# NVlabs/STEP

Hardware: AMD Instinct MI355X
Metric: clips_per_sec_T32_224 (higher is better)
Workload: dtype bf16; 1 GPU; C2: I3D backbone (BaseNet conv3d_1a..mixed_4f) forward, 8 x [3,32,224,224] clips per GPU, inputs resident in HBM, random-init weights; clips_per_gpu=8, T=32, HW=224, parallelism=clip-sharded replicas x1 (no data-path collective), batches_in_flight=2

## Files before the change

include/step_amd.h:

```cpp
#ifndef STEP_AMD_H
#define STEP_AMD_H

#include <stddef.h>
#include <stdint.h>

#ifdef __cplusplus
extern "C" {
#endif

#define STEP_API __attribute__((visibility("default")))

typedef void* step_stream_t;

enum { STEP_F32 = 0, STEP_BF16 = 1, STEP_F16 = 2 };
enum { STEP_NCHW = 0, STEP_NHWC = 1 };

enum {
    STEP_OK = 0,
    STEP_E_DTYPE = -1,
    STEP_E_SHAPE = -2,
    STEP_E_NULL = -3,
    STEP_E_UNSUPPORTED = -4,
    STEP_E_ALIGN = -5
};
// ... 8 lines not shown
STEP_API int step_hbm_stream_probe(const void* src, void* dst, size_t bytes, int workgroups, step_stream_t stream);

enum {
    STEP_OPT_CONV_IMPL = 0,
    STEP_OPT_CONV_NB,
    STEP_OPT_CONV_WAVES,
    STEP_OPT_CONV_PHASED,
    STEP_OPT_CONV_GEN,
    STEP_OPT_CONV_GMODE,
    STEP_OPT_CONV_PWS,
    STEP_OPT_CONV_SPLITK,
    STEP_OPT_CONV_TAIL,
    STEP_OPT_CONV_SLOTS,
    STEP_OPT_POOL_DIRECT,
    STEP_OPT_WGRAD_MINPIX,
    STEP_OPT_WGRAD16_LDS,
    STEP_OPT_CONV_GROUP_PW,
    STEP_OPT_CLIP_VEC,
    STEP_OPT_CONV_NB_RULE,
    STEP_OPT_THROUGHPUT,
    STEP_OPT_CONV_PERSIST,
    STEP_OPT_CONV_PWS_WAVES,
    STEP_OPT_CONV_GROUP_NARROW,
    STEP_OPT_COUNT_
};
STEP_API int step_set_option(int option, int value);
STEP_API int step_get_option(int option, int* value);
STEP_API void step_reset_options(void);
STEP_API const char* step_option_name(int option);

STEP_API int step_roi_align_forward(const void* feat, int dtype, int layout, const float* rois, int K, int B,
                                    int C, int H, int W, int pooled_h, int pooled_w, float spatial_scale,
                                    int sampling_ratio, void* out, step_stream_t stream);

STEP_API int step_roi_align_tubes_forward(const void* feat, int dtype, const float* rois, int K, int B, int T_all, int T, int C,
                                          int H, int W, int pooled_h, int pooled_w, float spatial_scale, int sampling_ratio,
                                          void* out, step_stream_t stream);

#define STEP_ROI_BWD_GATHER 0
#define STEP_ROI_BWD_ATOMIC 1
STEP_API int step_roi_align_backward(const float* grad, int layout, const float* rois, int K, int B, int C, int H,
                                     int W, int pooled_h, int pooled_w, float spatial_scale, int sampling_ratio,
                                     int mode, float* grad_feat, step_stream_t stream);

STEP_API int step_roi_pool_forward(const void* feat, int dtype, int layout, const float* rois, int K, int B, int C,
                                   int H, int W, int pooled_h, int pooled_w, float spatial_scale, void* out,
// ... 48 lines not shown
STEP_API size_t step_conv_packed_elems(int Cout, int Cin, int kd, int kh, int kw);
STEP_API int step_conv_pack_weight(const float* w, int Cout, int Cin, int kd, int kh, int kw, int dtype,
                                   const int32_t* perm_c, void* packed, step_stream_t stream);
STEP_API int step_conv_pack_weight_dgrad(const float* w, int Cout, int Cin, int kd, int kh, int kw, int dtype, int cin_pad,
                                         void* packed, step_stream_t stream);
typedef struct step_pack_item {
    const float* w;
    const int32_t* perm_c;
    void* packed;
    int Cout, Cin, w_cin, cin_lo;
    int kd, kh, kw;
    int dgrad, cin_pad;
    int reserved;
} step_pack_item;
STEP_API int step_conv_pack_weights(const step_pack_item* items, int n, int dtype, step_stream_t stream);
STEP_API int step_conv_forward(const step_conv_desc* d, const void* x, const void* w_packed, const float* scale,
                               const float* shift, const void* res, void* y, void* y2, step_stream_t stream);

STEP_API int step_pool_conv_forward(int dtype, const void* x, int N, int D, int H, int W, int C, int x_cstride, int x_coff, void* pool_y,
                                    int py_cstride, int py_coff, const step_conv_desc* d, const void* cx, const void* w_packed,
                                    const float* scale, const float* shift, void* y, void* y2, step_stream_t stream);

STEP_API int step_pool_conv_plan_nb(const step_conv_desc* d);

STEP_API int step_conv_forward_cat(const step_conv_desc* d, const void* x, int cin_a, const void* xb, int xb_cstride, int xb_coff,
                                   const void* w_packed, const float* scale, const float* shift, const void* res, void* y, void* y2,
                                   step_stream_t stream);

STEP_API int step_conv_forward_pre(const step_conv_desc* d, const void* x, const void* w_packed, const float* scale, const float* shift,
                                   const void* pre_w_packed, const float* pre_scale, const float* pre_shift, int pre_cin, void* y,
                                   step_stream_t stream);

STEP_API size_t step_conv_pre_pool_workspace_bytes(const step_conv_desc* d);
STEP_API int step_conv_forward_pre_pool(const step_conv_desc* d, const void* x, const void* w_packed, const float* scale, const float* shift,
                                        const void* pre_w_packed, const float* pre_scale, const float* pre_shift, int pre_cin, void* y_pooled,
                                        void* ws, size_t ws_bytes, step_stream_t stream);
STEP_API int step_conv_forward_pre_pool_tiles(const step_conv_desc* d, const void* x, const void* w_packed, const float* scale, const float* shift,
                                              const void* pre_w_packed, const float* pre_scale, const float* pre_shift, int pre_cin, void* y_pooled,
                                              void* ws, size_t ws_bytes, step_stream_t stream);
STEP_API int step_conv_pre_pool_finish(const step_conv_desc* d, void* y_pooled, void* ws, size_t ws_bytes, step_stream_t stream);

typedef struct step_conv_item {
    const step_conv_desc* desc;
    const void* x; const void* w_packed; const float* scale; const float* shift; const void* res; void* y;
} step_conv_item;
STEP_API int step_conv_forward_group(const step_conv_item* items, int n, step_stream_t stream);
// ... 227 lines not shown
```

step_amd/_capi.py:

```python
import ctypes as C

F32, BF16, F16 = 0, 1, 2
NCHW, NHWC = 0, 1
ROI_BWD_GATHER, ROI_BWD_ATOMIC = 0, 1
ABI_VERSION = 48

vp, fp, ip, u8p = C.c_void_p, C.c_void_p, C.c_void_p, C.c_void_p
i, f, ll, sz = C.c_int, C.c_float, C.c_longlong, C.c_size_t


class ConvDesc(C.Structure):
    _fields_ = [(n, C.c_int) for n in (
        "dtype", "N", "D", "H", "W", "Cin", "Cout", "kd", "kh", "kw", "x_cstride", "x_coff", "y_cstride", "y_coff",
        "res_cstride", "res_coff", "relu", "split", "y2_cstride", "y2_coff")]


class PackItem(C.Structure):
    _fields_ = [("w", C.c_void_p), ("perm_c", C.c_void_p), ("packed", C.c_void_p)] + [(n, C.c_int) for n in (
        "Cout", "Cin", "w_cin", "cin_lo", "kd", "kh", "kw", "dgrad", "cin_pad", "reserved")]


class ConvItem(C.Structure):
    _fields_ = [("desc", C.POINTER(ConvDesc)), ("x", C.c_void_p), ("w_packed", C.c_void_p), ("scale", C.c_void_p), ("shift", C.c_void_p),
                ("res", C.c_void_p), ("y", C.c_void_p)]


class WgradReduceItem(C.Structure):
    _fields_ = [("ws", C.c_void_p), ("dw", C.c_void_p), ("jobs", C.c_longlong)] + [(n, C.c_int) for n in (
# ... 16 lines not shown
    "step_roi_pool_backward": (i, [fp, ip, i, fp, i, i, i, i, i, i, i, fp, vp]),
    "step_mfma_clock_probe": (i, [vp, i, i, vp]),
    "step_hbm_stream_probe": (i, [vp, vp, sz, i, vp]),
    "step_clock_sample": (i, [vp, i, i, vp]),
    "step_nms_scratch_bytes": (sz, [i, i]),
    "step_nms_batched": (i, [fp, fp, ip, i, i, f, u8p, vp, vp]),
    "step_nms_batched_f64": (i, [fp, fp, ip, i, i, f, u8p, vp, vp]),
    "step_detect_compact": (i, [u8p, vp, vp, vp, ip, i, i, i, i, f, f, fp, fp, vp, vp, ip, vp]),
    "step_detect_merge": (i, [fp, ip, ip, ip, i, i, f, ip, ip, fp, ip, vp]),
    "step_round_sig4": (i, [fp, ll, fp, ip, vp]),
    "step_eval_match": (i, [fp, ip, vp, fp, ip, vp, i, ll, ll, i, C.c_double, u8p, ip, vp]),
    "step_eval_ap": (i, [vp, u8p, vp, i, ll, fp, fp, fp, vp]),
    "step_detect_nms": (i, [fp, ll, i, fp, ll, ip, ip, i, i, f, f, f, f, u8p, fp, vp]),
    "step_conv_packed_elems": (sz, [i, i, i, i, i]),
    "step_conv_pack_weight": (i, [fp, i, i, i, i, i, i, ip, vp, vp]),
    "step_conv_pack_weight_dgrad": (i, [fp, i, i, i, i, i, i, i, vp, vp]),
    "step_conv_pack_weights": (i, [vp, i, i, vp]),
    "step_conv_forward": (i, [C.POINTER(ConvDesc), vp, vp, fp, fp, vp, vp, vp, vp]),
    "step_conv_forward_group": (i, [C.POINTER(ConvItem), i, vp]),
    "step_conv_group_kernel_name": (i, [C.POINTER(ConvItem), i, C.c_char_p, i]),
    "step_conv_workspace_bytes": (sz, [C.POINTER(ConvDesc)]),
    "step_pool_conv_forward": (i, [i, vp, i, i, i, i, i, i, i, vp, i, i, C.POINTER(ConvDesc), vp, vp, fp, fp, vp, vp, vp]),
    "step_pool_conv_plan_nb": (i, [C.POINTER(ConvDesc)]),
    "step_conv_forward_cat": (i, [C.POINTER(ConvDesc), vp, i, vp, i, i, vp, fp, fp, vp, vp, vp, vp]),
    "step_conv_forward_pre": (i, [C.POINTER(ConvDesc), vp, vp, fp, fp, vp, fp, fp, i, vp, vp]),
    "step_conv_pre_pool_workspace_bytes": (sz, [C.POINTER(ConvDesc)]),
    "step_conv_forward_pre_pool": (i, [C.POINTER(ConvDesc), vp, vp, fp, fp, vp, fp, fp, i, vp, vp, sz, vp]),
    "step_conv_forward_pre_pool_tiles": (i, [C.POINTER(ConvDesc), vp, vp, fp, fp, vp, fp, fp, i, vp, vp, sz, vp]),
    "step_conv_pre_pool_finish": (i, [C.POINTER(ConvDesc), vp, vp, sz, vp]),
    "step_conv_wgrad": (i, [C.POINTER(ConvDesc), vp, fp, fp, i, vp]),
    "step_conv_wgrad_workspace_bytes": (sz, [C.POINTER(ConvDesc)]),
    "step_conv_wgrad_ws": (i, [C.POINTER(ConvDesc), vp, fp, fp, i, vp, sz, vp]),
    "step_conv_wgrad16": (i, [C.POINTER(ConvDesc), vp, vp, fp, i, vp]),
    "step_conv_wgrad16_workspace_bytes": (sz, [C.POINTER(ConvDesc)]),
    "step_conv_wgrad16_ws": (i, [C.POINTER(ConvDesc), vp, vp, fp, i, vp, sz, vp]),
    "step_conv_wgrad_kernel_name": (i, [C.POINTER(ConvDesc), i, C.c_char_p, i]),
    "step_conv_wgrad_partial": (i, [C.POINTER(ConvDesc), vp, vp, i, fp, i, vp, sz, C.POINTER(WgradReduceItem), vp]),
    "step_wgrad_reduce_group": (i, [C.POINTER(WgradReduceItem), i, vp]),
    "step_conv_forward_ws": (i, [C.POINTER(ConvDesc), vp, vp, fp, fp, vp, vp, vp, vp, sz, vp]),
    "step_conv_kernel_name": (i, [C.POINTER(ConvDesc), C.c_char_p, i]),
    "step_conv_plan_info": (i, [C.POINTER(ConvDesc), C.POINTER(C.c_int), i]),
    "step_conv_pre_pool_plan_info": (i, [C.POINTER(ConvDesc), C.POINTER(C.c_int), i]),
    "step_stem_packed_elems": (sz, [i]),
    "step_stem_pack_weight": (i, [fp, i, i, vp, vp]),
    "step_stem_forward": (i, [i, vp, i, i, i, i, vp, fp, fp, i, i, vp, i, i, vp]),
    "step_stem_pool_workspace_bytes": (sz, [i, i, i, i, i, i]),
# ... 50 lines not shown

def declare(lib, strict=True):
    for name, (res, args) in SIGNATURES.items():
        if not strict and not hasattr(lib, name):
            continue
        fn = getattr(lib, name)
        fn.restype = res
        fn.argtypes = args
    return lib


_ERR = {-1: "unsupported dtype", -2: "bad shape", -3: "null pointer", -4: "unsupported configuration",
        -5: "misaligned pointer or channel count"}


def check(status, what):
    if status != 0:
        msg = _ERR.get(status, "hipError_t %d" % status) if status < 0 else "hipError_t %d" % status
        raise RuntimeError("%s failed: %s" % (what, msg))


OPTION_IDS = {name: k for k, name in enumerate((
    "conv_impl", "conv_nb", "conv_waves", "conv_phased", "conv_gen", "conv_gmode", "conv_pws", "conv_splitk", "conv_tail",
    "conv_slots", "pool_direct", "wgrad_minpix", "wgrad16_lds", "conv_group_pw", "clip_vec", "conv_nb_rule", "throughput", "conv_persist", "conv_pws_waves", "conv_group_narrow"))}


def set_option(lib, name, value):
    check(lib.step_set_option(OPTION_IDS[name], int(value)), "step_set_option(%s, %r)" % (name, value))


def get_option(lib, name):
    v = C.c_int()
    check(lib.step_get_option(OPTION_IDS[name], C.byref(v)), "step_get_option(%s)" % name)
    return v.value


class options:

    def __init__(self, lib, **kw):
        self.lib, self.kw = lib, kw

    def __enter__(self):
        self.prev = {k: get_option(self.lib, k) for k in self.kw}
        for k, v in self.kw.items():
            set_option(self.lib, k, v)
        return self

# ... 5 lines not shown
```

step_amd/backbone.py:

```python
import os
import weakref

import torch
import torch.nn as nn

from . import ops, wgrad
from .wgrad import STATE as WGRAD, wgrad_into_grad, wgrad_sync

BN_EPS = 1e-5

MIXED_CFG = {
    "3b": (192, (64, 96, 128, 16, 32, 32)), "3c": (256, (128, 128, 192, 32, 96, 64)),
    "4b": (480, (192, 96, 208, 16, 48, 64)), "4c": (512, (160, 112, 224, 24, 64, 64)),
    "4d": (512, (128, 128, 256, 24, 64, 64)), "4e": (512, (112, 144, 288, 32, 64, 64)),
    "4f": (528, (256, 160, 320, 32, 128, 128)), "5b": (832, (256, 160, 320, 32, 128, 128)),
    "5c": (832, (384, 192, 384, 48, 128, 128)),
}


def _ver(*tensors):
    return tuple((t.data_ptr(), t._version, t.device) for t in tensors if t is not None)


class _ConvUnitFn(torch.autograd.Function):
# ... 650 lines not shown
        grad = torch.is_grad_enabled() and (x.requires_grad or any(p.requires_grad for p in self.parameters()))
        bn_train = any(u._unit.bn_training for u in (self.branch_0, self.branch_1[0], self.branch_1[1], self.branch_2[0], self.branch_2[1], self.branch_3[1]))
        if grad and not bn_train and self._train_fn_ok(x):
            u0, u1a, u1b, u2a, u2b, u3 = self._train_units()
            y = _MixedTrainFn.apply(x, u0.weight_fn(), u1a.weight_fn(), u1b.weight_fn(), u2a.weight_fn(), u2b.weight_fn(), u3.weight_fn(), self)
            if out is not None:
                out.copy_(y)
                return out
            return y
        if grad or bn_train:
            y = torch.cat([self.branch_0(x), self.branch_1[1](self.branch_1[0](x)), self.branch_2[1](self.branch_2[0](x)),
                           self.branch_3[1](self.branch_3[0](x))], dim=-1)
            if out is not None:
                out.copy_(y)
                return out
            return y
        if out is None:
            out = torch.empty((N, D, H, W, self.out_channels), dtype=x.dtype, device=x.device)
        c0, c1, c2 = oc[0], oc[0] + oc[2], oc[0] + oc[2] + oc[4]
        t = torch.empty((N, D, H, W, oc[1] + oc[3]), dtype=x.dtype, device=x.device)
        if BRANCH_STREAMS == 0 or not x.is_cuda:
            pool = self.branch_3[0]
            p = self._fused(x, out[..., :c0], t, pool=POOL_WITH_POINTWISE and pool.kernel_size == (3, 3, 3) and pool.stride == (1, 1, 1))
            if p is None:
                p = pool(x)
            u1, u2, u3 = self.branch_1[1]._unit, self.branch_2[1]._unit, self.branch_3[1]._unit
            m = []
            for u, xin, o in ((u1, t[..., :oc[1]], out[..., c0:c1]), (u2, t[..., oc[1]:], out[..., c1:c2]), (u3, p, out[..., c2:])):
                scale, shift = u.affine()
                m.append((xin, u.packed(x.dtype), u.cout, u.k, scale, None if shift is None else shift.detach().contiguous(), True, o))
            ops.conv_forward_group(m)
            return out
        main = torch.cuda.current_stream(x.device)
        s1, s2 = WGRAD.side_streams(x.device)
        if BRANCH_STREAMS == 1:
            s1 = s2
        s2.wait_stream(main)
        with torch.cuda.stream(s2):
            p = self._branch_3(x, out[..., c2:])
        self._fused(x, out[..., :c0], t)
        s1.wait_stream(main)
        with torch.cuda.stream(s1):
            self.branch_2[1](t[..., oc[1]:], out=out[..., c1:c2])
        self.branch_1[1](t[..., :oc[1]], out=out[..., c0:c1])
        main.wait_stream(s1)
        if s2 is not s1:
            main.wait_stream(s2)
        if p is not None:
            p.record_stream(main)
        return out

    def _branch_3(self, x, out):
        pool, unit = self.branch_3[0], self.branch_3[1]
        p = pool(x)
        unit(p, out=out)
        return p


POOL_WITH_POINTWISE = True
FUSE_STEM_POOL = True
FUSE_STEM_U8 = False
FUSE_CONV_POOL = True
FUSE_POINTWISE_INPUT = True


def _stem_then_pool(a, b, x, u8=None):
    if not (isinstance(a, Unit3D) and a.is_stem and isinstance(b, MaxPoolTF)) or not x.is_cuda or x.dtype == torch.float32:
        return None
    if b.kernel_size != (1, 3, 3) or b.stride != (1, 2, 2) or not a.relu or a._unit.bn_training or a._unit.bn is None:
        return None
    w = a.conv3d.weight
    bn = a.batch3d
    if torch.is_grad_enabled() and (w.requires_grad or bn.weight.requires_grad or bn.bias.requires_grad or x.requires_grad):
        return None
    scale, shift = a._unit.affine()
    if u8 is not None:
        dtype, mode, mean, std = u8
        return ops.stem_pool_forward_u8(x, dtype, a.stem_packed(dtype), w.shape[0], scale, shift, mode, mean, std)
    return ops.stem_pool_forward(x, a.stem_packed(x.dtype), w.shape[0], scale, shift)


def _pointwise_then_3x3x3(a, b, x, pool=None):
# ... 223 lines not shown
```

step_amd/csrc/conv_common.h:

```cpp
#pragma once
#include "options.h"
#include "common.h"
#include <stdio.h>
#include <stdlib.h>
#include <type_traits>
#include <utility>

namespace step {


constexpr int CK = 32;

__host__ __device__ constexpr int taps_padded(int ntaps) { return (ntaps > 1 && (ntaps & 1)) ? ntaps + 1 : ntaps; }

struct ConvParams {
    const void* x; const void* w; const float* scale; const float* shift; const void* res; void* y; void* y2;
    int split, y2_cstride, y2_coff;
    int N, D, H, W, Cin, Cout;
    int x_cstride, x_coff, y_cstride, y_coff, r_cstride, r_coff;
    int relu;
    int tiles_h, tiles_w, tiles_d;
    int gtd, gth, gtw;
    int gmode;
    int gx, gy;
    int gbase, gcount;
    int tile0;
    const void* x2; int x2_cstride, x2_coff, s_split;
    int gpersist;
    int narrow;
    int nchunks;
    int nchunks32;
    int vec_epi;
    int nblk32;
    long long Mtot;
    unsigned mag_hhw, mag_hw;
    const void* pre_w; const float* pre_scale; const float* pre_shift;
    void* pool_row; void* pool_col; int Hp, Wp;
    int pool_p2;
#ifdef STEP_PROBE
    unsigned long long* probe;
#endif
};

int pool333_pw_launch(int dtype, const void* x, int N, int D, int H, int W, int C, int x_cstride, int x_coff, void* y, int y_cstride, int y_coff,
                      ConvParams cp, long long conv_blocks, int nbc, step_stream_t stream);

constexpr int CONV_GROUP_MAX = 2;
struct ConvGroupParams { ConvParams p[CONV_GROUP_MAX]; int n; ConvParams pw; };

#ifdef STEP_PROBE
extern unsigned long long* g_probe_buf;
__device__ __forceinline__ void probe_mark(unsigned long long* probe, int slot) {
    if (probe && threadIdx.x == 0) probe[(size_t)blockIdx.x * 16 + slot] = __builtin_amdgcn_s_memrealtime();
}
__device__ __forceinline__ void probe_clock_begin(unsigned long long* probe) {
    if (probe && threadIdx.x == 0) probe[(size_t)blockIdx.x * 16 + 14] = __builtin_amdgcn_s_memtime();
}
__device__ __forceinline__ void probe_clock_end(unsigned long long* probe) {
    if (probe && threadIdx.x == 0) probe[(size_t)blockIdx.x * 16 + 14] = __builtin_amdgcn_s_memtime() - probe[(size_t)blockIdx.x * 16 + 14];
}
__device__ __forceinline__ void probe_ids(unsigned long long* probe) {
    probe_clock_begin(probe);
    if (probe && threadIdx.x == 0) {
        const unsigned hw = __builtin_amdgcn_s_getreg((31 << 11) | 4);
        const unsigned xcc = __builtin_amdgcn_s_getreg((31 << 11) | 20);
        probe[(size_t)blockIdx.x * 16 + 15] = ((unsigned long long)xcc << 32) | hw;
    }
}
#define STEP_PROBE_MARK(p, slot) probe_mark((p).probe, slot)
// ... 135 lines not shown
```

step_amd/csrc/conv_igemm.hip:

```cpp
#include "conv_common.h"

namespace step {

template <typename T, int TWL, int NB, int KD, int KH, int KW, bool FLAT, int CKT>
__global__ __launch_bounds__(256) void conv_igemm_kernel(ConvParams p) {
    constexpr int TW = 1 << TWL, TH = 128 >> TWL;
    constexpr int HH_ = TH + KH - 1, HW_ = TW + KW - 1;
    constexpr int NPIX = FLAT ? 128 : KD * HH_ * HW_;
    constexpr int ES = (int)sizeof(T);
    constexpr int VEC = 16 / ES;
    constexpr int PITCH = CKT * ES;
    constexpr int KSTEPS = CKT / 16;
    constexpr int SLOTS = PITCH / 16;
    constexpr int PPR = (16 / SLOTS) > 0 ? (16 / SLOTS) : 1;
    constexpr int NTAPS = KD * KH * KW;
    constexpr int NVEC = NPIX * SLOTS;
    constexpr int ITER = (NVEC + 255) / 256;
    typedef typename Ld16<T>::type vec16;
    typedef typename frag<T>::type frag_t;

    constexpr int LDSB = (NPIX * PITCH > 16384) ? NPIX * PITCH : 16384;
    __shared__ __attribute__((aligned(16))) unsigned char lds[LDSB];

    const int tid = threadIdx.x;
// ... 764 lines not shown
    step_conv_desc canon;
    ConvParams p;
    const int rc = conv_fill_params(d, cx, w_packed, scale, shift, nullptr, y, y2, canon, p);
    if (rc != STEP_OK) return rc;
    if (N == 0 && p.N == 0) return STEP_OK;
    if (!x || !pool_y) return STEP_E_NULL;
    if (N == 0 || p.N == 0 || canon.dtype != dtype || dtype == STEP_F32 || !(canon.kd == 1 && canon.kh == 1 && canon.kw == 1)) return STEP_E_UNSUPPORTED;
    constexpr int VEC = 8;
    if (canon.Cin % VEC || canon.x_cstride % VEC || canon.x_coff % VEC || ((uintptr_t)p.x % 16) || ((uintptr_t)p.w % 16) || ((uintptr_t)x % 16) ||
        ((uintptr_t)pool_y % 16))
        return STEP_E_UNSUPPORTED;
    const ConvPlan pl = conv_plan(&canon, false);
    if (!pl.ok || pl.impl != 2 || pl.NB > 2) return STEP_E_UNSUPPORTED;
    p.tiles_h = pl.tiles_h; p.tiles_w = pl.tiles_w; p.tiles_d = pl.tiles_d;
    p.gtd = pl.gtd; p.gth = pl.gth; p.gtw = pl.gtw; p.gmode = pl.gmode;
    const long long mtiles = ceil_div64(p.Mtot, 128);
    const int nbc = pool_conv_nbc(pl, p.Mtot, p.nblk32);
    const int groups = ceil_div(p.nblk32, 2 * nbc);
    p.gx = (int)mtiles; p.gy = groups;
    const long long tot = (mtiles * groups + 7) / 8 * 8;
    return pool333_pw_launch(dtype, x, N, D, H, W, C, x_cstride, x_coff, pool_y, py_cstride, py_coff, p, tot, nbc, stream);
}

int step_conv_forward_pre(const step_conv_desc* d, const void* x, const void* w_packed, const float* scale, const float* shift,
                          const void* pre_w_packed, const float* pre_scale, const float* pre_shift, int pre_cin, void* y, step_stream_t stream) {
    step_conv_desc canon;
    ConvParams p;
    const int rc = conv_fill_params(d, x, w_packed, scale, shift, nullptr, y, nullptr, canon, p);
    if (rc != STEP_OK) return rc;
    if (!pre_w_packed) return STEP_E_NULL;
    if (pre_cin != 64 || canon.Cin != 64 || canon.dtype == STEP_F32 || canon.split || !(canon.kd == 3 && canon.kh == 3 && canon.kw == 3))
        return STEP_E_UNSUPPORTED;
    if (((uintptr_t)pre_w_packed % 16) || (pre_scale && ((uintptr_t)pre_scale % 16)) || (pre_shift && ((uintptr_t)pre_shift % 16))) return STEP_E_ALIGN;
    if (p.N == 0) return STEP_OK;
    if ((unsigned long long)p.Mtot * (unsigned long long)canon.x_cstride >= 0xffffffffULL) return STEP_E_UNSUPPORTED;
    const ConvPlan pl = conv_plan(&canon);
    if (!pl.ok || pl.impl != 1 || pl.ph != 1 || pl.wv != 8 || pl.tps != 2 || (pl.twl != 0 && pl.twl != 3)) return STEP_E_UNSUPPORTED;
    p.pre_w = pre_w_packed; p.pre_scale = pre_scale; p.pre_shift = pre_shift;
    return canon.dtype == STEP_BF16 ? conv_forward_t<bf16_t>(&canon, p, nullptr, 0, stream) : conv_forward_t<f16_t>(&canon, p, nullptr, 0, stream);
}

}
namespace step {
struct PoolFixParams { void* y; const void* rowbuf; const void* colbuf; long long planes; int H, W, Hp, Wp, tiles_h, tiles_w, C, y_cstride, y_coff, PT; };
__global__ __launch_bounds__(256) void pool_seam_fix_kernel(PoolFixParams p) {
    const int nbr = p.tiles_h - 1, nbc = p.tiles_w - 1, PT = p.PT;
// ... 358 lines not shown
    step_conv_desc canon;
    ConvPlan pl;
    bool p2 = false;
    if (!conv_pre_pool_plan(d, canon, pl, p2)) return STEP_E_UNSUPPORTED;
    info[0] = pl.impl; info[1] = pl.twl; info[2] = pl.NB; info[3] = pl.wv; info[4] = pl.ph; info[5] = pl.gtd; info[6] = pl.gth; info[7] = pl.gtw;
    info[8] = pl.gmode; info[9] = (int)(pl.mtiles > 0x7fffffff ? 0x7fffffff : pl.mtiles);
    info[10] = pl.tiles_h; info[11] = pl.tiles_w;
    if (n >= 13) {
        const long long slots_ = opt(STEP_OPT_CONV_SLOTS) > 0 ? opt(STEP_OPT_CONV_SLOTS) : 256;
        long long main_tiles = pl.mtiles;
        const long long tail = pl.mtiles % slots_;
        const int tgroups = ceil_div(ceil_div(canon.Cout, 32), 2);
        if (opt(STEP_OPT_CONV_TAIL) != 0 && pl.NB > 1 && pl.mtiles > slots_ && tail > 0 && tail * 4 <= slots_ && tail * tgroups <= slots_) main_tiles -= tail;
        const bool one_group = ceil_div(ceil_div(canon.Cout, 32), 2 * pl.NB) == 1;
        info[12] = (opt(STEP_OPT_CONV_PERSIST) != 0 && one_group && pl.NB == 3 && main_tiles > slots_) ? (int)(slots_ / 8 * 8 > 0 ? slots_ / 8 * 8 : 8) : 0;
    }
    return STEP_OK;
}

#ifdef STEP_PROBE
__attribute__((visibility("default"))) void step_probe_set(void* buf) { step::g_probe_buf = (unsigned long long*)buf; }
#endif
const char* step_version(void) { return "step_amd 0.1.0 gfx950"; }
int step_abi_version(void) { return 48; }

}
```

step_amd/csrc/options.hip:

```cpp
#include <atomic>
#include <limits.h>

#include "options.h"

namespace step {

namespace {
struct OptSpec { const char* name; int def, lo, hi; };
constexpr OptSpec SPEC[STEP_OPT_COUNT_] = {
    {"conv_impl", -1, -1, 5},
    {"conv_nb", 0, 0, 3},
    {"conv_waves", 0, 0, 8},
    {"conv_phased", 2, 0, 2},
    {"conv_gen", 93, 0, 100},
    {"conv_gmode", 1, 0, 1},
    {"conv_pws", -1, -1, 1},
    {"conv_splitk", 1, 0, 1},
    {"conv_tail", 1, 0, 1},
    {"conv_slots", 0, 0, 1 << 20},
    {"pool_direct", 0, 0, 1},
    {"wgrad_minpix", 0, 0, 1 << 24},
    {"wgrad16_lds", 1, 0, 2},
    {"conv_group_pw", 1 << 20, 0, 1 << 20},
    {"clip_vec", 1, 0, 1},
    {"conv_nb_rule", 0, 0, 1},
    {"throughput", 0, 0, 1},
    {"conv_persist", 1, 0, 1},
    {"conv_pws_waves", 0, 0, 16},
    {"conv_group_narrow", 1, 0, 2},
};
std::atomic<int> g_delta[STEP_OPT_COUNT_];
}

int opt(int id) { return SPEC[id].def + g_delta[id].load(std::memory_order_relaxed); }

}

using namespace step;

extern "C" {

int step_set_option(int option, int value) {
    if (option < 0 || option >= STEP_OPT_COUNT_) return STEP_E_SHAPE;
    if (value < SPEC[option].lo || value > SPEC[option].hi) return STEP_E_SHAPE;
    if (option == STEP_OPT_CONV_WAVES && value != 0 && value != 4 && value != 8) return STEP_E_SHAPE;
    if (option == STEP_OPT_CONV_PWS_WAVES && value != 0 && value != 8 && value != 16) return STEP_E_SHAPE;
    if (option == STEP_OPT_CONV_IMPL && (value == 3 || value == 4)) return STEP_E_SHAPE;
    g_delta[option].store(value - SPEC[option].def, std::memory_order_relaxed);
    return STEP_OK;
}

int step_get_option(int option, int* value) {
// ... 16 lines not shown
```

step_amd/csrc/pool.hip:

```cpp
#include "common.h"
#include "conv_pw_kernel.h"
#include "pool_vec.h"
#include "options.h"
#include <stdlib.h>

namespace step {

__host__ __device__ static inline int tf_pad_front(int k, int s) { int a = k - s; if (a < 0) a = 0; return a / 2; }
__host__ __device__ static inline int tf_pad_total(int k, int s) { int a = k - s; return a < 0 ? 0 : a; }
__host__ __device__ static inline int pool_out_size(int L, int k, int s) {
    int Lp = L + tf_pad_total(k, s);
    int o = (Lp - k + s - 1) / s + 1;
    if ((o - 1) * s >= Lp) --o;
    return o;
}

struct PoolParams {
    int N, D, H, W, C, x_cstride, x_coff;
    int Do, Ho, Wo, y_cstride, y_coff;
    int kd, kh, kw, sd, sh, sw;
    int pfd, pfh, pfw;
    int Lpd, Lph, Lpw;
};

// ... 189 lines not shown
                *(raw*)(yn + (size_t)(w0p / SD) * yplane + hp_goffs[q]) = VecMax<T>::dec(m);
            }
            m2[q] = m1[q]; m1[q] = m0[q];
        }
    };
    raw rg[R];
    load_plane(pbeg, rg);
    for (int pd = pbeg; pd < pend; ++pd) step(pd, rg);
}

template <typename T, int KD, int KH, int KW, int SD, int SH, int SW, int NT>
__global__ __launch_bounds__(NT) void maxpool_sep_kernel(const T* __restrict__ x, T* __restrict__ y, PoolParams p,
                                                          int TH, int TW, int tiles_h, int tiles_w, int cchunks, int dseg, int nseg) {
    maxpool_sep_body<T, KD, KH, KW, SD, SH, SW, NT>(x, y, p, TH, TW, tiles_h, tiles_w, cchunks, dseg, nseg, (int)blockIdx.x, (int)gridDim.x);
}

template <typename T, int NBC = 1>
__global__ __launch_bounds__(256, NBC == 1 ? 3 : 2) void pool333_pw_kernel(const T* __restrict__ x, T* __restrict__ y, PoolParams p, int TH, int TW, int tiles_h,
                                                                           int tiles_w, int cchunks, int dseg, int nseg, int npool, ConvParams cp) {
    constexpr int ARENA = PP_LDS_BYTES > conv_pw_lds_bytes<T, NBC, 4>() ? PP_LDS_BYTES : conv_pw_lds_bytes<T, NBC, 4>();
    __shared__ __attribute__((aligned(16))) unsigned char arena[ARENA];
    if ((int)blockIdx.x < npool) maxpool_sep_body<T, 3, 3, 3, 1, 1, 1, 256, true>(x, y, p, TH, TW, tiles_h, tiles_w, cchunks, dseg, nseg, (int)blockIdx.x, npool, arena);
    else conv_pw_body<T, NBC, 4, true, 2>(cp, arena);
}

template <typename T>
__global__ void maxpool3d_tf_bwd_kernel(const T* __restrict__ x, const float* __restrict__ gy, float* __restrict__ gx, PoolParams p,
                                        long long total) {
    for (long long idx = (long long)blockIdx.x * blockDim.x + threadIdx.x; idx < total;
         idx += (long long)blockDim.x * gridDim.x) {
        const int c = (int)(idx % p.C);
        long long pix = idx / p.C;
        const int ow = (int)(pix % p.Wo); pix /= p.Wo;
        const int oh = (int)(pix % p.Ho); pix /= p.Ho;
        const int od = (int)(pix % p.Do);
        const int n = (int)(pix / p.Do);
        float best = -__builtin_inff();
        long long arg = -1;
        for (int a = 0; a < p.kd; ++a) {
            const int pd = od * p.sd + a;
            if (pd >= p.Lpd) break;
            const int id = pd - p.pfd;
            for (int b = 0; b < p.kh; ++b) {
                const int phh = oh * p.sh + b;
                if (phh >= p.Lph) break;
                const int ih = phh - p.pfh;
// ... 826 lines not shown
    p.kd = p.kh = p.kw = 3; p.sd = p.sh = p.sw = 1;
    p.pfd = p.pfh = p.pfw = tf_pad_front(3, 1);
    p.Lpd = D + tf_pad_total(3, 1); p.Lph = H + tf_pad_total(3, 1); p.Lpw = W + tf_pad_total(3, 1);
    const PoolSepPlan sp = pool_sep_plan(p, V);
    const long long npool = sp.blocks * sp.nseg;
    if (npool <= 0 || npool + conv_blocks > 0x7fffffffLL) return STEP_E_UNSUPPORTED;
    cp.gbase = (int)npool; cp.gcount = (int)conv_blocks;
    const dim3 grid((unsigned)(npool + conv_blocks));
    if (dtype == STEP_BF16 && nbc == 2)
        STEP_LAUNCH((pool333_pw_kernel<bf16_t, 2>), grid, dim3(256), stream, (const bf16_t*)x, (bf16_t*)y, p, sp.TH, sp.TW, sp.tiles_h, sp.tiles_w, sp.cchunks,
                    sp.dseg, sp.nseg, (int)npool, cp);
    else if (dtype == STEP_BF16)
        STEP_LAUNCH((pool333_pw_kernel<bf16_t>), grid, dim3(256), stream, (const bf16_t*)x, (bf16_t*)y, p, sp.TH, sp.TW, sp.tiles_h, sp.tiles_w, sp.cchunks,
                    sp.dseg, sp.nseg, (int)npool, cp);
    else if (nbc == 2)
        STEP_LAUNCH((pool333_pw_kernel<f16_t, 2>), grid, dim3(256), stream, (const f16_t*)x, (f16_t*)y, p, sp.TH, sp.TW, sp.tiles_h, sp.tiles_w, sp.cchunks,
                    sp.dseg, sp.nseg, (int)npool, cp);
    else
        STEP_LAUNCH((pool333_pw_kernel<f16_t>), grid, dim3(256), stream, (const f16_t*)x, (f16_t*)y, p, sp.TH, sp.TW, sp.tiles_h, sp.tiles_w, sp.cchunks,
                    sp.dseg, sp.nseg, (int)npool, cp);
    return STEP_LAUNCH_CHECK();
}

}

using namespace step;

extern "C" {

int step_pool_out_size(int L, int k, int s) { return pool_out_size(L, k, s); }

int step_maxpool3d_tf(int dtype, const void* x, int N, int D, int H, int W, int C, int x_cstride, int x_coff, int kd,
                      int kh, int kw, int sd, int sh, int sw, void* y, int y_cstride, int y_coff,
                      step_stream_t stream) {
    if (N < 0 || D <= 0 || H <= 0 || W <= 0 || C <= 0 || kd <= 0 || kh <= 0 || kw <= 0 || sd <= 0 || sh <= 0 || sw <= 0)
        return STEP_E_SHAPE;
    if (N == 0) return STEP_OK;
    if (!x || !y) return STEP_E_NULL;
    PoolParams p;
    p.N = N; p.D = D; p.H = H; p.W = W; p.C = C; p.x_cstride = x_cstride; p.x_coff = x_coff;
    p.Do = pool_out_size(D, kd, sd); p.Ho = pool_out_size(H, kh, sh); p.Wo = pool_out_size(W, kw, sw);
    p.y_cstride = y_cstride; p.y_coff = y_coff;
    p.kd = kd; p.kh = kh; p.kw = kw; p.sd = sd; p.sh = sh; p.sw = sw;
    p.pfd = tf_pad_front(kd, sd); p.pfh = tf_pad_front(kh, sh); p.pfw = tf_pad_front(kw, sw);
    p.Lpd = D + tf_pad_total(kd, sd); p.Lph = H + tf_pad_total(kh, sh); p.Lpw = W + tf_pad_total(kw, sw);
    switch (dtype) {
// ... 168 lines not shown
```

step_amd/ops.py:

```python
import ctypes

import torch

from . import _capi, _lib

DT = {torch.float32: _capi.F32, torch.bfloat16: _capi.BF16, torch.float16: _capi.F16}

PROFILE = None
PROFILE_LIMIT = None
WGRAD_WS = True
WGRAD16_WS = True


def _run(launch, describe, limited=True):
    if PROFILE is None:
        return launch()
    name, flops, nbytes = describe()
    if limited and PROFILE_LIMIT is not None:
        PROFILE.append((name, flops, nbytes, None, None))
        return launch() if len(PROFILE) <= PROFILE_LIMIT else None
    e0, e1 = torch.cuda.Event(enable_timing=True), torch.cuda.Event(enable_timing=True)
    e0.record()
    try:
        return launch()
# ... 171 lines not shown
    N, D, H, W, Cin = x.shape
    if x.dtype == torch.float32:
        return None
    d = _conv_desc(x, Cout, (1, 1, 1), _chan_slice(out), relu=relu, split=split, out2=out2)
    info = (ctypes.c_int * 10)()
    if L.step_conv_plan_info(ctypes.byref(d), info, 10) != 0 or info[0] != 2 or info[2] > POOL_CONV_MAX_NB:
        return None
    force = {"conv_nb": POOL_CONV_FORCE_NB} if POOL_CONV_FORCE_NB else {}
    with _capi.options(L, **force):
        nbc = L.step_pool_conv_plan_nb(ctypes.byref(d))
    if nbc <= 0:
        return None
    pooled = torch.empty((N, D, H, W, Cin), dtype=x.dtype, device=x.device)

    def describe():
        pix = N * D * H * W
        return ("void step::pool333_pw_kernel<%s, %d>(%s const*, %s*, step::PoolParams, int, int, int, int, int, int, int, int, step::ConvParams)" % (
            _TNAME[x.dtype], nbc, _TNAME[x.dtype], _TNAME[x.dtype]), 2.0 * pix * Cout * Cin, (pix * (3 * Cin + Cout) + Cout * Cin) * _ES[x.dtype])
    with _capi.options(L, **force):
        ran = _run_fused(lambda: L.step_pool_conv_forward(_dt(x), _lib.dptr(x), N, D, H, W, Cin, _chan_slice(x), 0, _lib.dptr(pooled), Cin, 0, ctypes.byref(d),
                                                          _lib.dptr(x), _lib.dptr(w_packed), _lib.dptr(scale), _lib.dptr(shift), _lib.dptr(out), _lib.dptr(out2),
                                                          _lib.stream_ptr(x.device)), describe, "step_pool_conv_forward")
    return pooled if ran else None


def conv_forward_pre(x, w_packed, Cout, k, scale, shift, relu, pre, out=None):
    L = _lib.lib()
    pw, pscale, pshift, cmid = pre
    N, D, H, W, Cpre = x.shape
    if out is None:
        out = torch.empty((N, D, H, W, Cout), dtype=x.dtype, device=x.device)
    d = _conv_desc(x, Cout, k, _chan_slice(out), cin=cmid, relu=relu)
    info = (ctypes.c_int * 10)()
    if Cpre != 64 or cmid != 64 or x.dtype == torch.float32 or tuple(k) != (3, 3, 3) or L.step_conv_plan_info(ctypes.byref(d), info, 10) != 0 \
            or not (info[0] == 1 and info[4] == 1 and info[3] == 8 and info[1] in (0, 3)):
        return None

    def describe():
        pix = N * D * H * W
        return ("void step::conv_tap_pre_kernel<%s, %d, %d>(step::ConvParams)" % (_TNAME[x.dtype], info[1], info[2]),
                2.0 * pix * (Cout * cmid * 27 + cmid * Cpre), (pix * (Cpre + Cout) + Cout * cmid * 27 + cmid * Cpre) * _ES[x.dtype])
    ran = _run_fused(lambda: L.step_conv_forward_pre(ctypes.byref(d), _lib.dptr(x), _lib.dptr(w_packed), _lib.dptr(scale), _lib.dptr(shift), _lib.dptr(pw),
                                                     _lib.dptr(pscale), _lib.dptr(pshift), int(Cpre), _lib.dptr(out), _lib.stream_ptr(x.device)),
                     describe, "step_conv_forward_pre")
    return out if ran else None

# ... 917 lines not shown
```

Measured before the change: 7601 clips/s.

## Fuse 3x3x3 maxpool with following pointwise conv in inception branch 3

Adds a kernel that computes the stride-1 3x3x3 max pool into LDS and feeds it straight into MFMA 1x1x1 convolution, so the pooled tensor is never written to HBM or read back. The inception block uses it when the existing pool+pointwise fusion did not run, then launches the other two branch convs as a group. Each tile now redoes the pooling halo work, and a heuristic gate on block count decides when the path applies, so fewer layers may qualify than expected.

```diff
diff --git a/include/step_amd.h b/include/step_amd.h
--- a/include/step_amd.h
+++ b/include/step_amd.h
@@ -54,6 +54,7 @@
     STEP_OPT_CONV_PERSIST,
     STEP_OPT_CONV_PWS_WAVES,
     STEP_OPT_CONV_GROUP_NARROW,
+    STEP_OPT_POOL_THEN_CONV,
     STEP_OPT_COUNT_
 };
 STEP_API int step_set_option(int option, int value);
@@ -148,6 +149,10 @@
                                     const float* scale, const float* shift, void* y, void* y2, step_stream_t stream);
 
 STEP_API int step_pool_conv_plan_nb(const step_conv_desc* d);
+
+STEP_API int step_pool_then_conv_forward(int dtype, const void* x, int N, int D, int H, int W, int x_cstride, int x_coff, const step_conv_desc* d,
+                                         const void* w_packed, const float* scale, const float* shift, void* y, step_stream_t stream);
+STEP_API int step_pool_then_conv_plan(const step_conv_desc* d);
 
 STEP_API int step_conv_forward_cat(const step_conv_desc* d, const void* x, int cin_a, const void* xb, int xb_cstride, int xb_coff,
                                    const void* w_packed, const float* scale, const float* shift, const void* res, void* y, void* y2,
diff --git a/step_amd/_capi.py b/step_amd/_capi.py
--- a/step_amd/_capi.py
+++ b/step_amd/_capi.py
@@ -3,7 +3,7 @@
 F32, BF16, F16 = 0, 1, 2
 NCHW, NHWC = 0, 1
 ROI_BWD_GATHER, ROI_BWD_ATOMIC = 0, 1
-ABI_VERSION = 48
+ABI_VERSION = 49
 
 vp, fp, ip, u8p = C.c_void_p, C.c_void_p, C.c_void_p, C.c_void_p
 i, f, ll, sz = C.c_int, C.c_float, C.c_longlong, C.c_size_t
@@ -66,6 +66,8 @@
     "step_conv_workspace_bytes": (sz, [C.POINTER(ConvDesc)]),
     "step_pool_conv_forward": (i, [i, vp, i, i, i, i, i, i, i, vp, i, i, C.POINTER(ConvDesc), vp, vp, fp, fp, vp, vp, vp]),
     "step_pool_conv_plan_nb": (i, [C.POINTER(ConvDesc)]),
+    "step_pool_then_conv_forward": (i, [i, vp, i, i, i, i, i, i, C.POINTER(ConvDesc), vp, fp, fp, vp, vp]),
+    "step_pool_then_conv_plan": (i, [C.POINTER(ConvDesc)]),
     "step_conv_forward_cat": (i, [C.POINTER(ConvDesc), vp, i, vp, i, i, vp, fp, fp, vp, vp, vp, vp]),
     "step_conv_forward_pre": (i, [C.POINTER(ConvDesc), vp, vp, fp, fp, vp, fp, fp, i, vp, vp]),
     "step_conv_pre_pool_workspace_bytes": (sz, [C.POINTER(ConvDesc)]),
@@ -162,7 +164,8 @@
 
 OPTION_IDS = {name: k for k, name in enumerate((
     "conv_impl", "conv_nb", "conv_waves", "conv_phased", "conv_gen", "conv_gmode", "conv_pws", "conv_splitk", "conv_tail",
-    "conv_slots", "pool_direct", "wgrad_minpix", "wgrad16_lds", "conv_group_pw", "clip_vec", "conv_nb_rule", "throughput", "conv_persist", "conv_pws_waves", "conv_group_narrow"))}
+    "conv_slots", "pool_direct", "wgrad_minpix", "wgrad16_lds", "conv_group_pw", "clip_vec", "conv_nb_rule", "throughput", "conv_persist", "conv_pws_waves", "conv_group_narrow",
+    "pool_then_conv"))}
 
 
 def set_option(lib, name, value):
diff --git a/step_amd/backbone.py b/step_amd/backbone.py
--- a/step_amd/backbone.py
+++ b/step_amd/backbone.py
@@ -696,13 +696,19 @@
         if BRANCH_STREAMS == 0 or not x.is_cuda:
             pool = self.branch_3[0]
             p = self._fused(x, out[..., :c0], t, pool=POOL_WITH_POINTWISE and pool.kernel_size == (3, 3, 3) and pool.stride == (1, 1, 1))
+            u1, u2, u3 = self.branch_1[1]._unit, self.branch_2[1]._unit, self.branch_3[1]._unit
+            def member(u, xin, o):
+                scale, shift = u.affine()
+                return (xin, u.packed(x.dtype), u.cout, u.k, scale, None if shift is None else shift.detach().contiguous(), True, o)
+            m = [member(u1, t[..., :oc[1]], out[..., c0:c1]), member(u2, t[..., oc[1]:], out[..., c1:c2])]
+            if p is None and POOL_THEN_POINTWISE and pool.kernel_size == (3, 3, 3) and pool.stride == (1, 1, 1):
+                b3 = member(u3, x, out[..., c2:])
+                if ops.pool_then_conv_forward(x, b3[1], b3[2], b3[4], b3[5], True, b3[7]) is not None:
+                    ops.conv_forward_group(m)
+                    return out
             if p is None:
                 p = pool(x)
-            u1, u2, u3 = self.branch_1[1]._unit, self.branch_2[1]._unit, self.branch_3[1]._unit
-            m = []
-            for u, xin, o in ((u1, t[..., :oc[1]], out[..., c0:c1]), (u2, t[..., oc[1]:], out[..., c1:c2]), (u3, p, out[..., c2:])):
-                scale, shift = u.affine()
-                m.append((xin, u.packed(x.dtype), u.cout, u.k, scale, None if shift is None else shift.detach().contiguous(), True, o))
+            m.append(member(u3, p, out[..., c2:]))
             ops.conv_forward_group(m)
             return out
         main = torch.cuda.current_stream(x.device)
@@ -732,6 +738,7 @@
 
 
 POOL_WITH_POINTWISE = True
+POOL_THEN_POINTWISE = True
 FUSE_STEM_POOL = True
 FUSE_STEM_U8 = False
 FUSE_CONV_POOL = True
diff --git a/step_amd/csrc/conv_common.h b/step_amd/csrc/conv_common.h
--- a/step_amd/csrc/conv_common.h
+++ b/step_amd/csrc/conv_common.h
@@ -45,6 +45,9 @@
 int pool333_pw_launch(int dtype, const void* x, int N, int D, int H, int W, int C, int x_cstride, int x_coff, void* y, int y_cstride, int y_coff,
                       ConvParams cp, long long conv_blocks, int nbc, step_stream_t stream);
 
+int pool333_then_pw_launch(int dtype, const void* x, int N, int D, int H, int W, int x_cstride, int x_coff, const ConvParams& cp, step_stream_t stream);
+long long pool333_then_pw_blocks(int N, int D, int H, int W);
+
 constexpr int CONV_GROUP_MAX = 2;
 struct ConvGroupParams { ConvParams p[CONV_GROUP_MAX]; int n; ConvParams pw; };
 
diff --git a/step_amd/csrc/conv_igemm.hip b/step_amd/csrc/conv_igemm.hip
--- a/step_amd/csrc/conv_igemm.hip
+++ b/step_amd/csrc/conv_igemm.hip
@@ -810,6 +810,45 @@
     return pool333_pw_launch(dtype, x, N, D, H, W, C, x_cstride, x_coff, pool_y, py_cstride, py_coff, p, tot, nbc, stream);
 }
 
+constexpr long long POOL_THEN_CONV_SLOTS = 512;
+static int pool_then_conv_nbc(const step_conv_desc* d) {
+    const int mode = opt(STEP_OPT_POOL_THEN_CONV);
+    if (!d || mode == 0 || (d->dtype != STEP_BF16 && d->dtype != STEP_F16) || !(d->kd == 1 && d->kh == 1 && d->kw == 1)) return 0;
+    if (d->N <= 0 || d->D <= 0 || d->H <= 0 || d->W <= 0 || d->Cin <= 0 || d->Cout <= 0) return 0;
+    if (d->Cin % 8 || d->Cin > 256 || d->Cout % 8 || d->Cout > 64 || (d->split > 0 && d->split < d->Cout)) return 0;
+    if (d->x_cstride % 8 || d->x_coff % 8 || d->y_cstride % 8 || d->y_coff % 8) return 0;
+    if ((long long)d->H * d->W * (d->x_cstride > d->y_cstride ? d->x_cstride : d->y_cstride) > 0x7fffffffLL) return 0;
+    const int nbc = ceil_div(d->Cout, 32);
+    if (mode == 1) {
+        const long long blocks = pool333_then_pw_blocks(d->N, d->D, d->H, d->W), rounds = ceil_div64(blocks, POOL_THEN_CONV_SLOTS);
+        if (blocks * 2 < POOL_THEN_CONV_SLOTS || blocks * 10 < rounds * POOL_THEN_CONV_SLOTS * 9) return 0;
+#ifdef STEP_EXP_PTP_ONLY_NBC
+        if (nbc != STEP_EXP_PTP_ONLY_NBC) return 0;
+#endif
+    }
+    return nbc;
+}
+
+int step_pool_then_conv_plan(const step_conv_desc* d) { return pool_then_conv_nbc(d); }
+
+int step_pool_then_conv_forward(int dtype, const void* x, int N, int D, int H, int W, int x_cstride, int x_coff, const step_conv_desc* d,
+                                const void* w_packed, const float* scale, const float* shift, void* y, step_stream_t stream) {
+    if (!d) return STEP_E_NULL;
+    if (N < 0 || D <= 0 || H <= 0 || W <= 0) return STEP_E_SHAPE;
+    if (d->N != N || d->D != D || d->H != H || d->W != W) return STEP_E_SHAPE;
+    if (x_coff < 0 || x_coff + d->Cin > x_cstride) return STEP_E_SHAPE;
+    if (d->split > 0 && d->split < d->Cout) return STEP_E_UNSUPPORTED;
+    step_conv_desc dx = *d;
+    dx.x_cstride = x_cstride; dx.x_coff = x_coff;
+    step_conv_desc canon;
+    ConvParams p;
+    const int rc = conv_fill_params(&dx, x, w_packed, scale, shift, nullptr, y, nullptr, canon, p);
+    if (rc != STEP_OK || p.N == 0) return rc;
+    if (dtype != d->dtype || pool_then_conv_nbc(&dx) == 0) return STEP_E_UNSUPPORTED;
+    if (((uintptr_t)x % 16) || ((uintptr_t)w_packed % 16) || ((uintptr_t)y % 16)) return STEP_E_ALIGN;
+    return pool333_then_pw_launch(dtype, x, N, D, H, W, x_cstride, x_coff, p, stream);
+}
+
 int step_conv_forward_pre(const step_conv_desc* d, const void* x, const void* w_packed, const float* scale, const float* shift,
                           const void* pre_w_packed, const float* pre_scale, const float* pre_shift, int pre_cin, void* y, step_stream_t stream) {
     step_conv_desc canon;
@@ -1214,6 +1253,6 @@
 __attribute__((visibility("default"))) void step_probe_set(void* buf) { step::g_probe_buf = (unsigned long long*)buf; }
 #endif
 const char* step_version(void) { return "step_amd 0.1.0 gfx950"; }
-int step_abi_version(void) { return 48; }
-
-}
+int step_abi_version(void) { return 49; }
+
+}
diff --git a/step_amd/csrc/options.hip b/step_amd/csrc/options.hip
--- a/step_amd/csrc/options.hip
+++ b/step_amd/csrc/options.hip
@@ -28,6 +28,7 @@
     {"conv_persist", 1, 0, 1},
     {"conv_pws_waves", 0, 0, 16},
     {"conv_group_narrow", 1, 0, 2},
+    {"pool_then_conv", 1, 0, 2},
 };
 std::atomic<int> g_delta[STEP_OPT_COUNT_];
 }
diff --git a/step_amd/csrc/pool.hip b/step_amd/csrc/pool.hip
--- a/step_amd/csrc/pool.hip
+++ b/step_amd/csrc/pool.hip
@@ -235,6 +235,195 @@
     __shared__ __attribute__((aligned(16))) unsigned char arena[ARENA];
     if ((int)blockIdx.x < npool) maxpool_sep_body<T, 3, 3, 3, 1, 1, 1, 256, true>(x, y, p, TH, TW, tiles_h, tiles_w, cchunks, dseg, nseg, (int)blockIdx.x, npool, arena);
     else conv_pw_body<T, NBC, 4, true, 2>(cp, arena);
+}
+
+constexpr int PTP_MAXKC16 = 16;
+constexpr int PTP_NG = 2;
+template <int NBC> constexpr int ptp_lds_bytes() { return PP_LDS_BYTES + NBC * PTP_MAXKC16 * 1024 + 2 * NBC * 32 * 4; }
+
+template <typename T, int NBC>
+__global__ __launch_bounds__(256, 2) void pool333_then_pw_kernel(const T* __restrict__ x, PoolParams p, int TH, int TW, int tiles_h, int tiles_w,
+                                                                 int dseg, int nseg, ConvParams cp) {
+    static_assert(sizeof(T) == 2, "16-bit storage types");
+    constexpr int V = 8, SL = PP_SL, R = PP_R, NT = 256, NG = PTP_NG;
+    static_assert(R * NT == PP_MAXIN * PP_MAXIN * SL, "one load item per 16-byte vector of the input tile");
+    typedef u16x8 raw;
+    typedef typename frag<T>::type frag_t;
+    __shared__ __attribute__((aligned(16))) unsigned char lds[ptp_lds_bytes<NBC>()];
+    raw* const lds_raw = (raw*)lds;
+    raw* const lds_w = lds_raw + R * NT;
+    unsigned char* const wl = lds + PP_LDS_BYTES;
+    float* const scl = (float*)(wl + NBC * PTP_MAXKC16 * 1024);
+    float* const shl = scl + NBC * 32;
+
+    const int tid = threadIdx.x, lane = tid & 63, khalf = lane >> 5;
+#ifdef STEP_EMUL
+    const int wave = tid >> 6;
+#else
+    const int wave = __builtin_amdgcn_readfirstlane(tid >> 6);
+#endif
+    const int nch = cp.nchunks32, KC16 = 2 * nch;
+    {
+        const u32x4* src = (const u32x4*)cp.w;
+        const int nv = NBC * KC16 * 64;
+        for (int v = tid; v < nv; v += NT) ((u32x4*)wl)[v] = src[v];
+        for (int i = tid; i < NBC * 32; i += NT) {
+            scl[i] = (cp.scale && i < cp.Cout) ? cp.scale[i] : 1.f;
+            shl[i] = (cp.shift && i < cp.Cout) ? cp.shift[i] : 0.f;
+        }
+    }
+
+    int t = (int)blockIdx.x;
+    const int nblk = (int)gridDim.x;
+    if ((nblk & 7) == 0) t = (t & 7) * (nblk >> 3) + (t >> 3);
+    const int tw_i = t % tiles_w; t /= tiles_w;
+    const int th_i = t % tiles_h; t /= tiles_h;
+    const int seg = t % nseg;
+    const int n = t / nseg;
+    const int oh0 = th_i * TH, ow0 = tw_i * TW;
+    const int IR = TH + 2, IC = TW + 2;
+    const int n_ld = IR * IC * SL, n_wp = IR * TW * SL, npix = TH * TW;
+
+    raw zero;
+#pragma unroll
+    for (int i = 0; i < V; ++i) zero[i] = 0;
+    const raw klow = VecMax<T>::lowest();
+
+    int ld_goff[R];
+    int wp_off[R], wp_dst[R];
+#pragma unroll
+    for (int q = 0; q < R; ++q) {
+        const int item = tid + q * NT;
+        const int sl = item & (SL - 1), pix = item / SL;
+        {
+            const int r = pix / IC, cl = pix % IC;
+            const int pr = oh0 + r, pc = ow0 + cl;
+            const int ih = pr - p.pfh, iw = pc - p.pfw;
+            ld_goff[q] = item >= n_ld ? -3 : ((pr >= p.Lph || pc >= p.Lpw) ? -2
+                       : ((ih >= 0 && ih < p.H && iw >= 0 && iw < p.W) ? (ih * p.W + iw) * p.x_cstride + p.x_coff + sl * V : -1));
+        }
+        {
+            const int r = pix / TW, ow = pix % TW;
+            wp_off[q] = item < n_wp ? (r * IC + ow) * SL + sl : -1;
+            wp_dst[q] = (pix * SL) | (sl ^ ((pix >> 2) & 3));
+        }
+    }
+    int hp_pix[NG], hp_yoff[NG];
+#pragma unroll
+    for (int gi = 0; gi < NG; ++gi) {
+        const int pix = (wave + 4 * gi) * 32 + (lane & 31);
+        const int oh = pix / TW, ow = pix % TW;
+        const int gh = oh0 + oh, gw = ow0 + ow;
+        const bool ok = pix < npix && gh < p.Ho && gw < p.Wo;
+        hp_pix[gi] = ok ? pix : -1;
+        hp_yoff[gi] = ok ? (gh * p.Wo + gw) * cp.y_cstride + cp.y_coff : -1;
+    }
+    const int ngroups = (npix + 31) >> 5;
+    const size_t xplane = (size_t)p.H * p.W * p.x_cstride, yplane = (size_t)p.Ho * p.Wo * cp.y_cstride;
+    const T* const xn = x + (size_t)n * p.D * xplane;
+    T* const yn = (T*)cp.y + (size_t)n * p.Do * yplane;
+
+    const int obeg = seg * dseg, oend = min(obeg + dseg, p.Do);
+    raw rg[3][R];
+    auto load_chunk = [&](int od, int ch) {
+#pragma unroll
+        for (int a = 0; a < 3; ++a) {
+            const int d = od + a - p.pfd;
+            const bool real = od < oend && d >= 0 && d < p.D;
+#pragma unroll
+            for (int q = 0; q < R; ++q) {
+                raw val = zero;
+                if (real && ld_goff[q] >= 0 && ch * 32 + ((tid + q * NT) & (SL - 1)) * V < p.C)
+                    val = *(const raw*)(xn + (size_t)d * xplane + ld_goff[q] + ch * 32);
+                rg[a][q] = val;
+            }
+        }
+    };
+
+    f32x16 acc[NG][NBC];
+#pragma unroll
+    for (int gi = 0; gi < NG; ++gi)
+#pragma unroll
+        for (int i = 0; i < NBC; ++i)
+#pragma unroll
+            for (int r = 0; r < 16; ++r) acc[gi][i][r] = 0.f;
+
+    load_chunk(obeg, 0);
+    for (int od = obeg; od < oend; ++od) {
+        for (int ch = 0; ch < nch; ++ch) {
+#pragma unroll
+            for (int q = 0; q < R; ++q)
+                if (ld_goff[q] != -3) {
+                    raw m = klow;
+                    if (ld_goff[q] != -2) m = VecMax<T>::max(VecMax<T>::max(VecMax<T>::enc(rg[0][q]), VecMax<T>::enc(rg[1][q])), VecMax<T>::enc(rg[2][q]));
+                    lds_raw[tid + q * NT] = m;
+                }
+            __syncthreads();
+            if (ch + 1 < nch) load_chunk(od, ch + 1);
+            else load_chunk(od + 1, 0);
+#pragma unroll
+            for (int q = 0; q < R; ++q)
+                if (wp_off[q] >= 0) {
+                    const raw* s0 = lds_raw + wp_off[q];
+                    lds_w[wp_dst[q]] = VecMax<T>::max(VecMax<T>::max(s0[0], s0[SL]), s0[2 * SL]);
+                }
+            __syncthreads();
+#pragma unroll
+            for (int gi = 0; gi < NG; ++gi) {
+                if (wave + 4 * gi >= ngroups) continue;
+                frag_t xf[2];
+#pragma unroll
+                for (int j = 0; j < 2; ++j) {
+                    raw m = zero;
+                    if (hp_pix[gi] >= 0) {
+                        const int sl = 2 * j + khalf;
+                        const int p0 = hp_pix[gi], p1 = p0 + TW, p2 = p1 + TW;
+                        m = VecMax<T>::max(VecMax<T>::max(lds_w[(p0 * SL) | (sl ^ ((p0 >> 2) & 3))], lds_w[(p1 * SL) | (sl ^ ((p1 >> 2) & 3))]),
+                                           lds_w[(p2 * SL) | (sl ^ ((p2 >> 2) & 3))]);
+                        m = VecMax<T>::dec(m);
+                    }
+                    xf[j] = m;
+                }
+#pragma unroll
+                for (int j = 0; j < 2; ++j)
+#pragma unroll
+                    for (int i = 0; i < NBC; ++i)
+                        mma_k16(lds_read_bfrag<T>(wl + ((size_t)(i * KC16 + 2 * ch + j) * 64 + lane) * 16), xf[j], acc[gi][i], T());
+            }
+        }
+#pragma unroll
+        for (int gi = 0; gi < NG; ++gi) {
+            if (wave + 4 * gi >= ngroups) continue;
+#pragma unroll
+            for (int i = 0; i < NBC; ++i) {
+                unsigned d[4][2];
+#pragma unroll
+                for (int q = 0; q < 4; ++q) {
+                    const int c4 = i * 32 + 8 * q + 4 * khalf;
+                    const f32x4 s4 = *(const f32x4*)(scl + c4), h4 = *(const f32x4*)(shl + c4);
+                    float v[4];
+#pragma unroll
+                    for (int e = 0; e < 4; ++e) {
+                        v[e] = acc[gi][i][4 * q + e] * s4[e] + h4[e];
+                        if (cp.relu) v[e] = relu_nan(v[e]);
+                        acc[gi][i][4 * q + e] = 0.f;
+                    }
+                    d[q][0] = (unsigned)elem<T>::bits16(v[0]) | ((unsigned)elem<T>::bits16(v[1]) << 16);
+                    d[q][1] = (unsigned)elem<T>::bits16(v[2]) | ((unsigned)elem<T>::bits16(v[3]) << 16);
+                }
+#pragma unroll
+                for (int h = 0; h < 2; ++h) {
+                    lane32_swap(d[2 * h][0], d[2 * h + 1][0]);
+                    lane32_swap(d[2 * h][1], d[2 * h + 1][1]);
+                    const int co = i * 32 + 16 * h + 8 * khalf;
+                    if (hp_yoff[gi] >= 0 && co < cp.Cout) {
+                        const u32x4 o = {d[2 * h][0], d[2 * h][1], d[2 * h + 1][0], d[2 * h + 1][1]};
+                        *(u32x4*)(yn + (size_t)od * yplane + hp_yoff[gi] + co) = o;
+                    }
+                }
+            }
+        }
+    }
 }
 
 template <typename T>
@@ -1107,6 +1296,48 @@
     return STEP_LAUNCH_CHECK();
 }
 
+#ifndef STEP_EXP_PTP_DSEG
+#define STEP_EXP_PTP_DSEG 1
+#endif
+static void pool333_then_pw_shape(int D, int H, int W, int& TH, int& TW, int& tiles_h, int& tiles_w, int& dseg, int& nseg) {
+    tiles_h = ceil_div(H, 14); tiles_w = ceil_div(W, 14);
+    TH = ceil_div(H, tiles_h); TW = ceil_div(W, tiles_w);
+    dseg = STEP_EXP_PTP_DSEG;
+    nseg = ceil_div(D, dseg);
+}
+long long pool333_then_pw_blocks(int N, int D, int H, int W) {
+    int TH, TW, th, tw, dseg, nseg;
+    pool333_then_pw_shape(D, H, W, TH, TW, th, tw, dseg, nseg);
+    return (long long)N * th * tw * nseg;
+}
+
+template <typename T>
+static void pool333_then_pw_launch_t(const void* x, const PoolParams& p, int TH, int TW, int tiles_h, int tiles_w, int dseg, int nseg, const ConvParams& cp,
+                                     dim3 grid, step_stream_t stream) {
+    if (cp.nblk32 == 1) STEP_LAUNCH((pool333_then_pw_kernel<T, 1>), grid, dim3(256), stream, (const T*)x, p, TH, TW, tiles_h, tiles_w, dseg, nseg, cp);
+    else STEP_LAUNCH((pool333_then_pw_kernel<T, 2>), grid, dim3(256), stream, (const T*)x, p, TH, TW, tiles_h, tiles_w, dseg, nseg, cp);
+}
+
+int pool333_then_pw_launch(int dtype, const void* x, int N, int D, int H, int W, int x_cstride, int x_coff, const ConvParams& cp, step_stream_t stream) {
+    PoolParams p;
+    p.N = N; p.D = D; p.H = H; p.W = W; p.C = cp.Cin; p.x_cstride = x_cstride; p.x_coff = x_coff;
+    p.Do = D; p.Ho = H; p.Wo = W;
+    p.y_cstride = cp.y_cstride; p.y_coff = cp.y_coff;
+    p.kd = p.kh = p.kw = 3; p.sd = p.sh = p.sw = 1;
+    p.pfd = p.pfh = p.pfw = tf_pad_front(3, 1);
+    p.Lpd = D + tf_pad_total(3, 1); p.Lph = H + tf_pad_total(3, 1); p.Lpw = W + tf_pad_total(3, 1);
+    int TH, TW, tiles_h, tiles_w, dseg, nseg;
+    pool333_then_pw_shape(D, H, W, TH, TW, tiles_h, tiles_w, dseg, nseg);
+    const long long blocks = (long long)N * tiles_h * tiles_w * nseg;
+    if (blocks <= 0 || blocks > 0x7fffffffLL || cp.nblk32 < 1 || cp.nblk32 > 2 || cp.nchunks32 * 2 > PTP_MAXKC16) return STEP_E_UNSUPPORTED;
+    if (TH < 1 || TW < 1 || TH > PP_MAXIN - 2 || TW > PP_MAXIN - 2) return STEP_E_UNSUPPORTED;
+    const dim3 grid((unsigned)blocks);
+    if (dtype == STEP_BF16) pool333_then_pw_launch_t<bf16_t>(x, p, TH, TW, tiles_h, tiles_w, dseg, nseg, cp, grid, stream);
+    else if (dtype == STEP_F16) pool333_then_pw_launch_t<f16_t>(x, p, TH, TW, tiles_h, tiles_w, dseg, nseg, cp, grid, stream);
+    else return STEP_E_UNSUPPORTED;
+    return STEP_LAUNCH_CHECK();
+}
+
 }
 
 using namespace step;
diff --git a/step_amd/ops.py b/step_amd/ops.py
--- a/step_amd/ops.py
+++ b/step_amd/ops.py
@@ -217,6 +217,26 @@
                                                           _lib.dptr(x), _lib.dptr(w_packed), _lib.dptr(scale), _lib.dptr(shift), _lib.dptr(out), _lib.dptr(out2),
                                                           _lib.stream_ptr(x.device)), describe, "step_pool_conv_forward")
     return pooled if ran else None
+
+
+def pool_then_conv_forward(x, w_packed, Cout, scale, shift, relu, out):
+    L = _lib.lib()
+    N, D, H, W, Cin = x.shape
+    if x.dtype == torch.float32 or not hasattr(L, "step_pool_then_conv_plan"):
+        return None
+    d = _conv_desc(x, Cout, (1, 1, 1), _chan_slice(out), relu=relu)
+    nbc = L.step_pool_then_conv_plan(ctypes.byref(d))
+    if nbc <= 0:
+        return None
+
+    def describe():
+        pix = N * D * H * W
+        return ("void step::pool333_then_pw_kernel<%s, %d>(%s const*, step::PoolParams, int, int, int, int, int, int, step::ConvParams)" % (
+            _TNAME[x.dtype], nbc, _TNAME[x.dtype]), 2.0 * pix * Cin * Cout, (pix * (Cin + Cout) + Cin * Cout) * _ES[x.dtype])
+    ran = _run_fused(lambda: L.step_pool_then_conv_forward(_dt(x), _lib.dptr(x), N, D, H, W, _chan_slice(x), 0, ctypes.byref(d), _lib.dptr(w_packed),
+                                                           _lib.dptr(scale), _lib.dptr(shift), _lib.dptr(out), _lib.stream_ptr(x.device)),
+                     describe, "step_pool_then_conv_forward")
+    return out if ran else None
 
 
 def conv_forward_pre(x, w_packed, Cout, k, scale, shift, relu, pre, out=None):
```

After: 7776 clips/s, median of 6. +2.3%, better.
